# seung-lab/chunkflow

Measured on AMD Instinct MI355X. Metric: output_voxels_per_sec, higher is better.
Workload: dtype f32; 1 GPU; config2-512cube-rsunet-affinity; batch_size=12, engine=rsunet

## Files before the change

chunkflow_amd/csrc/updown.hip:

```cpp
#include <hip/hip_runtime.h>
#include <hip/hip_bf16.h>

#include <algorithm>

#include "cfx_internal.h"

namespace {

typedef __hip_bfloat16 cfx_bf16;

template <typename T>
__device__ __forceinline__ float ldf(const T* p);
template <>
__device__ __forceinline__ float ldf<float>(const float* p) { return *p; }
template <>
__device__ __forceinline__ float ldf<cfx_bf16>(const cfx_bf16* p) {
    return __bfloat162float(*p);
}
__device__ __forceinline__ float cvf(float v) { return v; }
__device__ __forceinline__ float cvf(cfx_bf16 v) {
    return __bfloat162float(v);
}

template <typename T>
struct vec4;
template <>
struct vec4<float> {
    typedef float type __attribute__((ext_vector_type(4)));
    static __device__ __forceinline__ float get(type v, int i) {
        return v[i];
    }
};
template <>
struct vec4<cfx_bf16> {
    typedef unsigned short type __attribute__((ext_vector_type(4)));
    static __device__ __forceinline__ float get(type v, int i) {
        return __bfloat162float(
            __hip_bfloat16(__hip_bfloat16_raw{(unsigned short)v[i]}));
    }
};
template <typename T>
__device__ __forceinline__ void stf(T* p, float v);
template <>
__device__ __forceinline__ void stf<float>(float* p, float v) { *p = v; }
template <>
__device__ __forceinline__ void stf<cfx_bf16>(cfx_bf16* p, float v) {
    *p = __float2bfloat16(v);
}

template <typename T>
__device__ __forceinline__ void stage_rows(
    float* s_in, const T* in, const long long* row_off, int rows, int xn,
    int xvalid, int C, int CPAD, int tid, int nthreads) {
    const int total = rows * xn * C;
    for (int idx = tid; idx < total; idx += nthreads) {
        const int c = idx % C;
        const int x = (idx / C) % xn;
        const int r = idx / (C * xn);
        const float v = x < xvalid
                            ? ldf(&in[row_off[r] + (long long)x * C + c])
                            : 0.f;
        s_in[(r * xn + x) * CPAD + c] = v;
    }
}

template <typename T, int XI>
__global__ __launch_bounds__(256, 2) void k_upconv2(
    const T* __restrict__ in, const T* __restrict__ wgt,
    const float* __restrict__ bias, T* __restrict__ out, int N, int D,
    int H, int W, int C, int K) {
    constexpr int PX = XI / 8;
    extern __shared__ float smem[];
    float* s_w = smem;
    float* s_in = smem + C * K * 4;
    const int CPAD = C | 1;
    const int tid = threadIdx.x;
    const int kslot = tid & 31;
    const int pslot = tid >> 5;

    for (int idx = tid; idx < C * K * 4; idx += 256) {
        const int q = idx & 3;
        const int k = (idx >> 2) % K;
        const int c = (idx >> 2) / K;
        s_w[(c * K + k) * 4 + q] = ldf(&wgt[(q * C + c) * K + k]);
    }

    const int nz = blockIdx.z;
    const int y = blockIdx.y;
    const int x0 = blockIdx.x * XI;
    const int xvalid = min(XI, W - x0);
    long long row_off[1] = {((((long long)nz * H) + y) * W + x0) * C};
    stage_rows(s_in, in, row_off, 1, XI, xvalid, C, CPAD, tid, 256);
    __syncthreads();

    const long long out_base =
        ((((long long)nz * 2 * H) + 2 * y) * 2 * W) * K;

    for (int k = kslot; k < K; k += 32) {
        const float bj = bias ? bias[k] : 0.f;
        float acc[PX][4];
#pragma unroll
        for (int p = 0; p < PX; ++p)
#pragma unroll
            for (int q = 0; q < 4; ++q) acc[p][q] = bj;
        for (int c = 0; c < C; ++c) {
            const float4 w4 =
                *reinterpret_cast<const float4*>(&s_w[(c * K + k) * 4]);
#pragma unroll
            for (int p = 0; p < PX; ++p) {
                const float v = s_in[(pslot + p * 8) * CPAD + c];
                acc[p][0] += v * w4.x;
                acc[p][1] += v * w4.y;
                acc[p][2] += v * w4.z;
                acc[p][3] += v * w4.w;
            }
        }
#pragma unroll
        for (int p = 0; p < PX; ++p) {
            const int xi = x0 + pslot + p * 8;
            if (xi >= W) continue;
            T* op = out + out_base + (long long)2 * xi * K + k;
            stf(op, acc[p][0]);
            stf(op + K, acc[p][1]);
            stf(op + (long long)2 * W * K, acc[p][2]);
            stf(op + (long long)2 * W * K + K, acc[p][3]);
        }
    }
}


constexpr int UM_NW = 4;

typedef float um_f32x4 __attribute__((ext_vector_type(4)));

template <int NT, bool SKIP>
__global__ __launch_bounds__(UM_NW * 64) void k_upconv2_mfma(
    const float* __restrict__ in, const float* __restrict__ wgt,
    const float* __restrict__ bias, const float* __restrict__ skip,
    float* __restrict__ out, int W, int C, int xtiles, int ntiles) {
    constexpr int K = 4 * NT;
    constexpr int N4 = 4 * K;
    constexpr int BS = N4 + 4;
    constexpr int RUN4 = 2 * NT;
    extern __shared__ __attribute__((aligned(16))) float um_smem[];
    const int S = C >> 2;
    const int tid = threadIdx.x;
    const int lane = tid & 63;
    const int wave = __builtin_amdgcn_readfirstlane(tid >> 6);
    float* s_w = um_smem;
    float* s_b = um_smem + C * N4 + wave * (16 * BS);

    for (int idx = tid; idx < C * N4; idx += UM_NW * 64) {
        const int l = idx & 63;
        const int st = idx >> 6;
        const int t = st % NT;
        const int s = st / NT;
        const int c = 4 * s + (l >> 4);
        const int col = 16 * t + (l & 15);
        const int q = col / K;
        s_w[idx] = wgt[(q * C + c) * K + (col - q * K)];
    }
    __syncthreads();

    const int ai = lane & 15;
    const int akk = lane >> 4;
    float bj[NT];
#pragma unroll
    for (int t = 0; t < NT; ++t)
        bj[t] = bias ? bias[(16 * t + ai) % K] : 0.f;

    auto piece = [&](int it, int& py, int& i, int& j4) {
        const int f = it * 64 + lane;
        py = f >= 16 * RUN4;
        const int rem = f - py * (16 * RUN4);
        i = rem / RUN4;
        j4 = rem - i * RUN4;
    };
    auto a_loads = [&](int tile, float (&a)[16]) {
        const int xt = tile % xtiles;
        const long long row = tile / xtiles;
        const int x0 = xt * 16;
        const int ilast = min(16, W - x0) - 1;
        const float* ip = in + (row * W + x0) * C;
        const unsigned ao = min(ai, ilast) * C + akk;
#pragma unroll
        for (int s = 0; s < 16; ++s) a[s] = ip[ao + 4u * min(s, S - 1)];
    };
    auto skip_loads = [&](int tile, um_f32x4 (&sv)[NT]) {
        const int xt = tile % xtiles;
        const long long row = tile / xtiles;
        const int x0 = xt * 16;
        const int ilast = min(16, W - x0) - 1;
        const float* sp = skip + (2 * row * 2 * W + 2 * x0) * K;
#pragma unroll
        for (int it = 0; it < NT; ++it) {
            int py, i, j4;
            piece(it, py, i, j4);
            const unsigned so =
                py * (2 * W * K) + min(i, ilast) * (2 * K) + 4 * j4;
            sv[it] = *reinterpret_cast<const um_f32x4*>(sp + so);
        }
    };

    auto do_tile = [&](int tile, int next, const float (&a)[16],
                       float (&a2)[16]) {
        um_f32x4 sv[NT];
        if (SKIP) skip_loads(tile, sv);
        a_loads(next, a2);
        __builtin_amdgcn_sched_barrier(0);
        um_f32x4 acc[NT];
#pragma unroll
        for (int t = 0; t < NT; ++t)
            acc[t] = um_f32x4{bj[t], bj[t], bj[t], bj[t]};
#pragma unroll
        for (int s = 0; s < 16; ++s) {
            if (s >= S) break;
#pragma unroll
            for (int t = 0; t < NT; ++t)
                acc[t] = __builtin_amdgcn_mfma_f32_16x16x4f32(
                    a[s], s_w[(s * NT + t) * 64 + lane], acc[t], 0, 0, 0);
        }
#pragma unroll
        for (int t = 0; t < NT; ++t)
#pragma unroll
            for (int r = 0; r < 4; ++r)
                s_b[(akk * 4 + r) * BS + 16 * t + ai] = acc[t][r];
        __builtin_amdgcn_wave_barrier();

        const int xt = tile % xtiles;
        const long long row = tile / xtiles;
        const int x0 = xt * 16;
        const int nvalid = min(16, W - x0);
        float* op = out + (2 * row * 2 * W + 2 * x0) * K;
        um_f32x4 v[NT];
#pragma unroll
        for (int it = 0; it < NT; ++it) {
            int py, i, j4;
            piece(it, py, i, j4);
            v[it] = *reinterpret_cast<const um_f32x4*>(
                &s_b[i * BS + py * (2 * K) + 4 * j4]);
            if (SKIP) v[it] += sv[it];
        }
        __builtin_amdgcn_sched_barrier(0);
#pragma unroll
        for (int it = 0; it < NT; ++it) {
            int py, i, j4;
            piece(it, py, i, j4);
            const unsigned oo = py * (2 * W * K) + i * (2 * K) + 4 * j4;
            if (nvalid == 16 || i < nvalid)
                *reinterpret_cast<um_f32x4*>(op + oo) = v[it];
        }
        __builtin_amdgcn_wave_barrier();
    };

    const int stride = gridDim.x * UM_NW;
    int tile = blockIdx.x * UM_NW + wave;
    if (tile >= ntiles) return;
    float a0[16], a1[16];
    a_loads(tile, a0);
    while (true) {
        do_tile(tile, min(tile + stride, ntiles - 1), a0, a1);
        tile += stride;
        if (tile >= ntiles) break;
        do_tile(tile, min(tile + stride, ntiles - 1), a1, a0);
        tile += stride;
        if (tile >= ntiles) break;
    }
}

template <typename T, int XO>
__global__ __launch_bounds__(256, 2) void k_downconv2(
    const T* __restrict__ in, const T* __restrict__ wgt,
    const float* __restrict__ bias, T* __restrict__ out, int N, int D,
    int H, int W, int C, int K) {
    constexpr int PX = XO / 8;
    extern __shared__ float smem[];
    float* s_w = smem;
    float* s_in = smem + C * K * 4;
    const int CPAD = C | 1;
    const int tid = threadIdx.x;
    const int kslot = tid & 31;
    const int pslot = tid >> 5;
    const int HO = H >> 1, WO = W >> 1;

    for (int idx = tid; idx < C * K * 4; idx += 256) {
        const int q = idx & 3;
        const int k = (idx >> 2) % K;
        const int c = (idx >> 2) / K;
        s_w[(c * K + k) * 4 + q] = ldf(&wgt[(q * C + c) * K + k]);
    }

    const int nz = blockIdx.z;
    const int y = blockIdx.y;
    const int x0 = blockIdx.x * XO;
    const int xvalid = min(2 * XO, W - 2 * x0);
    long long row_off[2] = {
        ((((long long)nz * H) + 2 * y) * W + 2 * x0) * C,
        ((((long long)nz * H) + 2 * y + 1) * W + 2 * x0) * C};
    stage_rows(s_in, in, row_off, 2, 2 * XO, xvalid, C, CPAD, tid, 256);
    __syncthreads();

    const long long out_row = (((long long)nz * HO) + y) * WO * K;

    for (int k = kslot; k < K; k += 32) {
        const float bj = bias ? bias[k] : 0.f;
        float acc[PX];
#pragma unroll
        for (int p = 0; p < PX; ++p) acc[p] = bj;
        for (int c = 0; c < C; ++c) {
            const float4 w4 =
                *reinterpret_cast<const float4*>(&s_w[(c * K + k) * 4]);
#pragma unroll
            for (int p = 0; p < PX; ++p) {
                const int xl = 2 * (pslot + p * 8);
                acc[p] += s_in[xl * CPAD + c] * w4.x;
                acc[p] += s_in[(xl + 1) * CPAD + c] * w4.y;
                acc[p] += s_in[(2 * XO + xl) * CPAD + c] * w4.z;
                acc[p] += s_in[(2 * XO + xl + 1) * CPAD + c] * w4.w;
            }
        }
#pragma unroll
        for (int p = 0; p < PX; ++p) {
            const int xo = x0 + pslot + p * 8;
            if (xo >= WO) continue;
            stf(&out[out_row + (long long)xo * K + k], acc[p]);
        }
    }
}

template <typename T, int XI, int KC>
__global__ __launch_bounds__(256, 2) void k_conv155_c1(
    const T* __restrict__ in, const T* __restrict__ wgt,
    const float* __restrict__ bias, T* __restrict__ out, int N, int D,
    int H, int W, int K_rt) {
    const int K = KC > 0 ? KC : K_rt;
    __shared__ float s_in[5][XI + 4];
    __shared__ float s_w[32 * 28];
    const int tid = threadIdx.x;
    const int nz = blockIdx.z;
    const int y = blockIdx.y;
    const int x0 = blockIdx.x * XI;

    const long long plane = (long long)nz * H;
    for (int idx = tid; idx < 5 * (XI + 4); idx += XI) {
        const int dy = idx / (XI + 4);
        const int xl = idx % (XI + 4);
        const int gy = y + dy - 2;
        const int gx = x0 + xl - 2;
        const bool ok = gy >= 0 && gy < H && gx >= 0 && gx < W;
        s_in[dy][xl] = ok ? ldf(&in[(plane + gy) * W + gx]) : 0.f;
    }
    for (int idx = tid; idx < K * 28; idx += XI) {
        const int t = idx % 28;
        const int k = idx / 28;
        s_w[idx] = t < 25 ? ldf(&wgt[k * 25 + t]) : 0.f;
    }
    __syncthreads();

    const int gx = x0 + tid;
    if (gx >= W) return;
    float v[25];
#pragma unroll
    for (int dy = 0; dy < 5; ++dy)
#pragma unroll
        for (int dx = 0; dx < 5; ++dx)
            v[dy * 5 + dx] = s_in[dy][tid + dx];
    T* op = out + (plane + y) * (long long)W * K + (long long)gx * K;
    if (KC > 0 && KC % 4 == 0) {
        typedef unsigned int uint2v __attribute__((ext_vector_type(2)));
        typedef float float2v __attribute__((ext_vector_type(2)));
#pragma unroll 1
        for (int k = 0; k < KC; k += 4) {
            float a0 = bias ? bias[k] : 0.f;
            float a1 = bias ? bias[k + 1] : 0.f;
            float a2 = bias ? bias[k + 2] : 0.f;
            float a3 = bias ? bias[k + 3] : 0.f;
#pragma unroll
            for (int t4 = 0; t4 < 24; t4 += 4) {
                const float4 w0 = *reinterpret_cast<const float4*>(
                    &s_w[k * 28 + t4]);
                const float4 w1 = *reinterpret_cast<const float4*>(
                    &s_w[(k + 1) * 28 + t4]);
                const float4 w2 = *reinterpret_cast<const float4*>(
                    &s_w[(k + 2) * 28 + t4]);
                const float4 w3 = *reinterpret_cast<const float4*>(
                    &s_w[(k + 3) * 28 + t4]);
                a0 += v[t4] * w0.x + v[t4 + 1] * w0.y + v[t4 + 2] * w0.z +
                      v[t4 + 3] * w0.w;
                a1 += v[t4] * w1.x + v[t4 + 1] * w1.y + v[t4 + 2] * w1.z +
                      v[t4 + 3] * w1.w;
                a2 += v[t4] * w2.x + v[t4 + 1] * w2.y + v[t4 + 2] * w2.z +
                      v[t4 + 3] * w2.w;
                a3 += v[t4] * w3.x + v[t4 + 1] * w3.y + v[t4 + 2] * w3.z +
                      v[t4 + 3] * w3.w;
            }
            a0 += v[24] * s_w[k * 28 + 24];
            a1 += v[24] * s_w[(k + 1) * 28 + 24];
            a2 += v[24] * s_w[(k + 2) * 28 + 24];
            a3 += v[24] * s_w[(k + 3) * 28 + 24];
            if (sizeof(T) == 2) {
                uint2v u;
                u.x = (unsigned)((__hip_bfloat16_raw)__float2bfloat16(
                          a0)).x |
                      ((unsigned)((__hip_bfloat16_raw)__float2bfloat16(
                           a1)).x << 16);
                u.y = (unsigned)((__hip_bfloat16_raw)__float2bfloat16(
                          a2)).x |
                      ((unsigned)((__hip_bfloat16_raw)__float2bfloat16(
                           a3)).x << 16);
                *reinterpret_cast<uint2v*>(reinterpret_cast<char*>(op) +
                                           (size_t)k * 2) = u;
            } else {
                float2v f01, f23;
                f01.x = a0;
                f01.y = a1;
                f23.x = a2;
                f23.y = a3;
                float2v* d =
                    reinterpret_cast<float2v*>(reinterpret_cast<char*>(op) +
                                               (size_t)k * 4);
                d[0] = f01;
                d[1] = f23;
            }
        }
    } else {
        for (int k = 0; k < K; ++k) {
            float acc = bias ? bias[k] : 0.f;
#pragma unroll
            for (int t4 = 0; t4 < 24; t4 += 4) {
                const float4 w4 =
                    *reinterpret_cast<const float4*>(&s_w[k * 28 + t4]);
                acc += v[t4] * w4.x + v[t4 + 1] * w4.y +
                       v[t4 + 2] * w4.z + v[t4 + 3] * w4.w;
            }
            acc += v[24] * s_w[k * 28 + 24];
            stf(&op[k], acc);
        }
    }
}

constexpr int CO_R = 6;
constexpr int CO_S = 60;
constexpr int CO_PS = 72;

typedef float co_f32x4 __attribute__((ext_vector_type(4)));

__device__ __forceinline__ unsigned short bf16_bits(float v) {
    return ((__hip_bfloat16_raw)__float2bfloat16(v)).x;
}

template <typename T>
__global__ __launch_bounds__(256, 2) void k_conv155_out_mfma(
    const T* __restrict__ in, const float* __restrict__ wfrag,
    const float* __restrict__ bias, T* __restrict__ out, int H, int W,
    int vec_ok) {
    constexpr int RS = CO_R + 4;
    constexpr int XS = 64;
    constexpr int CC = 28, C4 = CC / 4;
    constexpr int NV = RS * XS * C4;
    constexpr int PER = (NV + 255) / 256;
    constexpr int BATCH = 6;
    static_assert(CO_R * 16 * CO_PS * 4 <= RS * XS * CC * (int)sizeof(T),
                  "P bounce must fit over the input tile");
    __shared__ __attribute__((aligned(16))) T s_in[RS * XS * CC];
    float* s_p = reinterpret_cast<float*>(s_in);

    const int tid = threadIdx.x;
    const int wave = tid >> 6;
    const int lane = tid & 63;
    const int y0 = blockIdx.y * CO_R;
    const int x0 = blockIdx.x * CO_S;
    const long long plane = (long long)blockIdx.z * H;
    const int nout = min(CO_S, W - x0);
    const int ntile = (nout + 4 + 15) >> 4;

    float b[35];
#pragma unroll
    for (int s = 0; s < 35; ++s) b[s] = wfrag[s * 64 + lane];

    typedef typename vec4<T>::type tx4;
#pragma unroll 1
    for (int b0 = 0; b0 < PER; b0 += BATCH) {
        tx4 v[BATCH];
#pragma unroll
        for (int u = 0; u < BATCH; ++u) {
            const int idx = (b0 + u) * 256 + tid;
            const int r = idx / (XS * C4);
            const int rem = idx - r * (XS * C4);
            const int xl = rem / C4;
            const int c4 = rem - xl * C4;
            const int gy = y0 + r - 2;
            const int gx = x0 + xl - 2;
            const bool ok = b0 + u < PER && idx < NV && gy >= 0 &&
                            gy < H && gx >= 0 && gx < W &&
                            xl < ntile * 16;
            v[u] = ok ? *reinterpret_cast<const tx4*>(
                            &in[((plane + gy) * W + gx) * (long long)CC +
                                c4 * 4])
                      : tx4{};
        }
#pragma unroll
        for (int u = 0; u < BATCH; ++u) {
            const int idx = (b0 + u) * 256 + tid;
            if (b0 + u < PER && idx < NV)
                *reinterpret_cast<tx4*>(&s_in[idx * 4]) = v[u];
        }
    }
    __syncthreads();

    co_f32x4 acc[CO_R];
#pragma unroll
    for (int y = 0; y < CO_R; ++y) acc[y] = co_f32x4{0.f, 0.f, 0.f, 0.f};
    if (wave < ntile) {
        const T* abase = &s_in[(wave * 16 + (lane & 15)) * CC + (lane >> 4)];
#pragma unroll
        for (int r = 0; r < RS; ++r) {
            float a[C4];
#pragma unroll
            for (int s = 0; s < C4; ++s)
                a[s] = cvf(abase[r * XS * CC + s * 4]);
#pragma unroll
            for (int s = 0; s < C4; ++s)
#pragma unroll
                for (int dy = 0; dy < 5; ++dy) {
                    const int y = r - dy;
                    if (y >= 0 && y < CO_R)
                        acc[y] = __builtin_amdgcn_mfma_f32_16x16x4f32(
                            a[s], b[dy * C4 + s], acc[y], 0, 0, 0);
                }
        }
    }
    __syncthreads();

    if (wave < ntile) {
#pragma unroll
        for (int y = 0; y < CO_R; ++y)
            *reinterpret_cast<co_f32x4*>(
                &s_p[(y * 16 + (lane & 15)) * CO_PS + wave * 16 +
                     (lane >> 4) * 4]) = acc[y];
    }
    __syncthreads();

    if (tid >= CO_R * (CO_S / 4)) return;
    const int yl = tid / (CO_S / 4);
    const int q = tid - yl * (CO_S / 4);
    const int y = y0 + yl;
    const int gx = x0 + q * 4;
    if (y >= H || gx >= W) return;
    float o[4][3];
#pragma unroll
    for (int e = 0; e < 4; ++e)
#pragma unroll
        for (int k = 0; k < 3; ++k) o[e][k] = bias ? bias[k] : 0.f;
#pragma unroll
    for (int j = 0; j < 15; ++j) {
        const int dx = j / 3, k = j % 3;
        const float* pr = &s_p[(yl * 16 + j) * CO_PS + q * 4];
        const co_f32x4 lo = *reinterpret_cast<const co_f32x4*>(pr);
        const co_f32x4 hi = *reinterpret_cast<const co_f32x4*>(pr + 4);
        const float p8[8] = {lo[0], lo[1], lo[2], lo[3],
                             hi[0], hi[1], hi[2], hi[3]};
#pragma unroll
        for (int e = 0; e < 4; ++e) o[e][k] += p8[e + dx];
    }
    T* op = out + ((plane + y) * W + gx) * 3LL;
    if (vec_ok) {
        if (sizeof(T) == 2) {
            typedef unsigned co_u32x2 __attribute__((ext_vector_type(2)));
            unsigned short h[12];
#pragma unroll
            for (int i = 0; i < 12; ++i) h[i] = bf16_bits(o[i / 3][i % 3]);
#pragma unroll
            for (int i = 0; i < 3; ++i) {
                co_u32x2 u;
                u.x = h[4 * i] | ((unsigned)h[4 * i + 1] << 16);
                u.y = h[4 * i + 2] | ((unsigned)h[4 * i + 3] << 16);
                reinterpret_cast<co_u32x2*>(op)[i] = u;
            }
        } else {
#pragma unroll
            for (int i = 0; i < 3; ++i) {
                co_f32x4 f;
#pragma unroll
                for (int m = 0; m < 4; ++m)
                    f[m] = o[(4 * i + m) / 3][(4 * i + m) % 3];
                reinterpret_cast<co_f32x4*>(op)[i] = f;
            }
        }
    } else {
#pragma unroll
        for (int e = 0; e < 4; ++e)
            if (gx + e < W)
#pragma unroll
                for (int k = 0; k < 3; ++k) stf(&op[e * 3 + k], o[e][k]);
    }
}

__device__ __forceinline__ float bre_act(float v, int do_elu) {
    if (do_elu) {
        const float e = expm1f(v > 0.f ? 0.f : v);
        v = v > 0.f ? v : e;
    }
    return v;
}

template <bool VEC>
__global__ __launch_bounds__(256) void k_bias_res_elu(
    float* __restrict__ y, const float* __restrict__ bias,
    const float* __restrict__ res, long long total, int K, int do_elu) {
    const long long step = (long long)gridDim.x * 256;
    long long i = (long long)blockIdx.x * 256 + threadIdx.x;
    if (VEC) {
        const long long n4 = total >> 2;
        const int K4 = K >> 2;
        for (; i < n4; i += step) {
            const int k4 = (int)(i % K4);
            um_f32x4 v = reinterpret_cast<const um_f32x4*>(y)[i];
            if (bias) v += reinterpret_cast<const um_f32x4*>(bias)[k4];
            if (res) v += reinterpret_cast<const um_f32x4*>(res)[i];
#pragma unroll
            for (int e = 0; e < 4; ++e) v[e] = bre_act(v[e], do_elu);
            reinterpret_cast<um_f32x4*>(y)[i] = v;
        }
    } else {
        for (; i < total; i += step) {
            float v = y[i];
            if (bias) v += bias[(int)(i % K)];
            if (res) v += res[i];
            y[i] = bre_act(v, do_elu);
        }
    }
}

}

extern "C" int cfx_conv155_out(cfx_ctx* ctx, const void* in,
                               const float* wfrag, const float* bias,
                               void* out, int N, int D, int H, int W,
                               int C, int K, int is_bf16) {
    if (C != 28 || K != 3) {
        g_err = "cfx_conv155_out: only C == 28, K == 3 instantiated";
        return -1;
    }
    if ((long long)N * D > 65535) {
        g_err = "cfx_conv155_out: N * D <= 65535 supported";
        return -1;
    }
    hipEvent_t e0;
    if (prof_begin(ctx, &e0)) return -1;
    dim3 grid((W + CO_S - 1) / CO_S, (H + CO_R - 1) / CO_R,
              (unsigned)(N * D));
    const int vec_ok = W % 4 == 0 && ((size_t)out & 15) == 0;
    if (is_bf16)
        hipLaunchKernelGGL((k_conv155_out_mfma<cfx_bf16>), grid, dim3(256),
                           0, ctx->stream, (const cfx_bf16*)in, wfrag, bias,
                           (cfx_bf16*)out, H, W, vec_ok);
    else
        hipLaunchKernelGGL((k_conv155_out_mfma<float>), grid, dim3(256), 0,
                           ctx->stream, (const float*)in, wfrag, bias,
                           (float*)out, H, W, vec_ok);
    CFX_CHECK(hipGetLastError());
    double flops = 2.0 * 25.0 * C * K * (double)N * D * H * W;
    if (prof_end(ctx, e0, CFX_K_CONV_STREAM, flops)) return -1;
    return 0;
}

extern "C" int cfx_conv155_c1(cfx_ctx* ctx, const void* in, const void* wgt,
                              const float* bias, void* out, int N, int D,
                              int H, int W, int K, int is_bf16) {
    if (K > 32) {
        g_err = "cfx_conv155_c1: K <= 32 supported";
        return -1;
    }
    constexpr int XI = 256;
    dim3 grid((W + XI - 1) / XI, H, (unsigned)(N * D));
    hipEvent_t e0;
    if (prof_begin(ctx, &e0)) return -1;
    if (is_bf16 && K == 28)
        hipLaunchKernelGGL((k_conv155_c1<cfx_bf16, XI, 28>), grid,
                           dim3(XI), 0, ctx->stream, (const cfx_bf16*)in,
                           (const cfx_bf16*)wgt, bias, (cfx_bf16*)out, N,
                           D, H, W, K);
    else if (is_bf16)
        hipLaunchKernelGGL((k_conv155_c1<cfx_bf16, XI, 0>), grid,
                           dim3(XI), 0, ctx->stream, (const cfx_bf16*)in,
                           (const cfx_bf16*)wgt, bias, (cfx_bf16*)out, N,
                           D, H, W, K);
    else if (K == 28)
        hipLaunchKernelGGL((k_conv155_c1<float, XI, 28>), grid, dim3(XI),
                           0, ctx->stream, (const float*)in,
                           (const float*)wgt, bias, (float*)out, N, D, H,
                           W, K);
    else
        hipLaunchKernelGGL((k_conv155_c1<float, XI, 0>), grid, dim3(XI),
                           0, ctx->stream, (const float*)in,
                           (const float*)wgt, bias, (float*)out, N, D, H,
                           W, K);
    CFX_CHECK(hipGetLastError());
    double flops = 2.0 * 25.0 * K * (double)N * D * H * W;
    if (prof_end(ctx, e0, CFX_K_CONV_STREAM, flops)) return -1;
    return 0;
}

namespace {

size_t um_shmem(int C, int K) {
    return ((size_t)C * 4 * K + (size_t)UM_NW * 16 * (4 * K + 4)) *
           sizeof(float);
}

bool um_eligible(const void* in, const void* skip, const void* out, int N,
                 int D, int H, int W, int C, int K) {
    return C % 4 == 0 && K % 4 == 0 && C >= 4 && C <= 64 && K >= 4 &&
           K <= 48 && (((size_t)in | (size_t)skip | (size_t)out) & 15) == 0 &&
           (long long)N * D * H * ((W + 15) / 16) < (1LL << 31);
}

template <int NT, bool SKIP>
int um_launch_nt(cfx_ctx* ctx, const float* in, const float* wgt,
                 const float* bias, const float* skip, float* out, int W,
                 int C, int xtiles, int ntiles) {
    const size_t shmem = um_shmem(C, 4 * NT);
    if (shmem > 64 * 1024)
        CFX_CHECK(hipFuncSetAttribute(
            reinterpret_cast<const void*>(&k_upconv2_mfma<NT, SKIP>),
            hipFuncAttributeMaxDynamicSharedMemorySize, (int)shmem));
    int cus = 0;
    CFX_CHECK(hipDeviceGetAttribute(
        &cus, hipDeviceAttributeMultiprocessorCount, ctx->device));
    const int per_cu = (int)std::min<size_t>(8, (160 * 1024) / shmem);
    const int grid =
        std::min((ntiles + UM_NW - 1) / UM_NW, std::max(1, cus * per_cu));
    hipLaunchKernelGGL((k_upconv2_mfma<NT, SKIP>), dim3(grid),
                       dim3(UM_NW * 64), shmem, ctx->stream, in, wgt, bias,
                       skip, out, W, C, xtiles, ntiles);
    CFX_CHECK(hipGetLastError());
    return 0;
}

template <bool SKIP>
int um_launch(cfx_ctx* ctx, const float* in, const float* wgt,
              const float* bias, const float* skip, float* out, int N,
              int D, int H, int W, int C, int K) {
    const int xtiles = (W + 15) / 16;
    const int ntiles = N * D * H * xtiles;
    if (ntiles == 0) return 0;
    switch (K / 4) {
#define UM_CASE(NT)                                                         \
    case NT:                                                                \
        return um_launch_nt<NT, SKIP>(ctx, in, wgt, bias, skip, out, W, C,  \
                                      xtiles, ntiles);
        UM_CASE(1) UM_CASE(2) UM_CASE(3) UM_CASE(4) UM_CASE(5) UM_CASE(6)
        UM_CASE(7) UM_CASE(8) UM_CASE(9) UM_CASE(10) UM_CASE(11)
        UM_CASE(12)
#undef UM_CASE
    }
    g_err = "upconv mfma: K not instantiated";
    return -1;
}

}

extern "C" int cfx_upconv_2x2_add(cfx_ctx* ctx, const void* in,
                                  const void* wgt, const float* bias,
                                  const void* skip, void* out, int N, int D,
                                  int H, int W, int C, int K, int is_bf16) {
    if (!skip)
        return cfx_upconv_2x2(ctx, in, wgt, bias, out, N, D, H, W, C, K,
                              is_bf16);
    if (is_bf16) {
        g_err = "cfx_upconv_2x2_add: skip is f32 only";
        return -1;
    }
    if (!um_eligible(in, skip, out, N, D, H, W, C, K)) {
        g_err = "cfx_upconv_2x2_add: skip needs C % 4 == 0, K % 4 == 0, "
                "C <= 64, K <= 48 and 16-byte aligned tensors";
        return -1;
    }
    hipEvent_t e0;
    if (prof_begin(ctx, &e0)) return -1;
    if (um_launch<true>(ctx, (const float*)in, (const float*)wgt, bias,
                        (const float*)skip, (float*)out, N, D, H, W, C, K))
        return -1;
    double flops = 2.0 * 4.0 * C * K * (double)N * D * H * W;
    if (prof_end(ctx, e0, CFX_K_CONV_STREAM, flops)) return -1;
    return 0;
}

extern "C" int cfx_upconv_2x2(cfx_ctx* ctx, const void* in, const void* wgt,
                              const float* bias, void* out, int N, int D,
                              int H, int W, int C, int K, int is_bf16) {
    if (K > 64 || C > 64) {
        g_err = "cfx_upconv_2x2: C, K <= 64 supported";
        return -1;
    }
    if (!is_bf16 && um_eligible(in, nullptr, out, N, D, H, W, C, K)) {
        hipEvent_t e0;
        if (prof_begin(ctx, &e0)) return -1;
        if (um_launch<false>(ctx, (const float*)in, (const float*)wgt, bias,
                             nullptr, (float*)out, N, D, H, W, C, K))
            return -1;
        double flops = 2.0 * 4.0 * C * K * (double)N * D * H * W;
        if (prof_end(ctx, e0, CFX_K_CONV_STREAM, flops)) return -1;
        return 0;
    }
    constexpr int XI = 64;
    dim3 grid((W + XI - 1) / XI, H, (unsigned)(N * D));
    const size_t shmem =
        ((size_t)C * K * 4 + (size_t)XI * (C | 1)) * sizeof(float);
    hipEvent_t e0;
    if (prof_begin(ctx, &e0)) return -1;
    if (is_bf16)
        hipLaunchKernelGGL((k_upconv2<cfx_bf16, XI>), grid, dim3(256),
                           shmem, ctx->stream, (const cfx_bf16*)in,
                           (const cfx_bf16*)wgt, bias, (cfx_bf16*)out, N, D,
                           H, W, C, K);
    else
        hipLaunchKernelGGL((k_upconv2<float, XI>), grid, dim3(256), shmem,
                           ctx->stream, (const float*)in, (const float*)wgt,
                           bias, (float*)out, N, D, H, W, C, K);
    CFX_CHECK(hipGetLastError());
    double flops = 2.0 * 4.0 * C * K * (double)N * D * H * W;
    if (prof_end(ctx, e0, CFX_K_CONV_STREAM, flops)) return -1;
    return 0;
}

extern "C" int cfx_downconv_2x2(cfx_ctx* ctx, const void* in,
                                const void* wgt, const float* bias,
                                void* out, int N, int D, int H, int W,
                                int C, int K, int is_bf16) {
    if (K > 64 || C > 64) {
        g_err = "cfx_downconv_2x2: C, K <= 64 supported";
        return -1;
    }
    if ((H | W) & 1) {
        g_err = "cfx_downconv_2x2: H, W must be even";
        return -1;
    }
    constexpr int XO = 64;
    dim3 grid((W / 2 + XO - 1) / XO, H / 2, (unsigned)(N * D));
    const size_t shmem =
        ((size_t)C * K * 4 + (size_t)2 * 2 * XO * (C | 1)) * sizeof(float);
    hipEvent_t e0;
    if (prof_begin(ctx, &e0)) return -1;
    if (is_bf16)
        hipLaunchKernelGGL((k_downconv2<cfx_bf16, XO>), grid, dim3(256),
                           shmem, ctx->stream, (const cfx_bf16*)in,
                           (const cfx_bf16*)wgt, bias, (cfx_bf16*)out, N, D,
                           H, W, C, K);
    else
        hipLaunchKernelGGL((k_downconv2<float, XO>), grid, dim3(256), shmem,
                           ctx->stream, (const float*)in, (const float*)wgt,
                           bias, (float*)out, N, D, H, W, C, K);
    CFX_CHECK(hipGetLastError());
    double flops = 2.0 * 4.0 * C * K * (double)N * D * (H / 2) * (W / 2);
    if (prof_end(ctx, e0, CFX_K_CONV_STREAM, flops)) return -1;
    return 0;
}

extern "C" int cfx_bias_res_elu(cfx_ctx* ctx, float* y, const float* bias,
                                const float* res, long long nvox, int K,
                                int do_elu) {
    if (nvox < 0 || K < 1) {
        g_err = "cfx_bias_res_elu: nvox >= 0, K >= 1";
        return -1;
    }
    const long long total = nvox * K;
    if (total == 0) return 0;
    const bool vec =
        K % 4 == 0 &&
        (((size_t)y | (size_t)bias | (size_t)res) & 15) == 0;
    const long long items = vec ? total / 4 : total;
    const int grid = (int)std::min<long long>((items + 255) / 256, 256 * 16);
    if (vec)
        hipLaunchKernelGGL((k_bias_res_elu<true>), dim3(grid), dim3(256), 0,
                           ctx->stream, y, bias, res, total, K, do_elu);
    else
        hipLaunchKernelGGL((k_bias_res_elu<false>), dim3(grid), dim3(256), 0,
                           ctx->stream, y, bias, res, total, K, do_elu);
    CFX_CHECK(hipGetLastError());
    return 0;
}
```

Baseline: 116.6 million voxels/s.

## Use MFMA for the 1-channel input conv and add y-walking fp32 output conv

After: 119.1 million voxels/s, median of 6. +2.2%, better.

```diff
diff --git a/chunkflow_amd/csrc/updown.hip b/chunkflow_amd/csrc/updown.hip
--- a/chunkflow_amd/csrc/updown.hip
+++ b/chunkflow_amd/csrc/updown.hip
@@ -46,6 +46,10 @@
 template <>
 __device__ __forceinline__ void stf<cfx_bf16>(cfx_bf16* p, float v) {
     *p = __float2bfloat16(v);
+}
+
+__device__ __forceinline__ unsigned short bf16_bits(float v) {
+    return ((__hip_bfloat16_raw)__float2bfloat16(v)).x;
 }
 
 template <typename T>
@@ -328,114 +332,143 @@
     }
 }
 
-template <typename T, int XI, int KC>
-__global__ __launch_bounds__(256, 2) void k_conv155_c1(
+constexpr int CI_R = 8;
+constexpr int CI_S = 64;
+constexpr int CI_NW = CI_S / 16;
+constexpr int CI_LW = CI_S + 4;
+
+template <typename T>
+__global__ __launch_bounds__(CI_NW * 64) void k_conv155_in_mfma(
     const T* __restrict__ in, const T* __restrict__ wgt,
-    const float* __restrict__ bias, T* __restrict__ out, int N, int D,
-    int H, int W, int K_rt) {
-    const int K = KC > 0 ? KC : K_rt;
-    __shared__ float s_in[5][XI + 4];
-    __shared__ float s_w[32 * 28];
+    const float* __restrict__ bias, T* __restrict__ out, int H, int W,
+    int K, int nstrips, int nrows, int vec_ok) {
+    constexpr int NS = (CI_R + 4) * CI_LW;
+    constexpr int PER = (NS + CI_NW * 64 - 1) / (CI_NW * 64);
+    __shared__ float s_in[NS];
+    __shared__ __attribute__((aligned(16))) float s_bounce[CI_NW][16 * 32];
+
     const int tid = threadIdx.x;
-    const int nz = blockIdx.z;
-    const int y = blockIdx.y;
-    const int x0 = blockIdx.x * XI;
-
-    const long long plane = (long long)nz * H;
-    for (int idx = tid; idx < 5 * (XI + 4); idx += XI) {
-        const int dy = idx / (XI + 4);
-        const int xl = idx % (XI + 4);
-        const int gy = y + dy - 2;
+    const int lane = tid & 63;
+    const int wave = __builtin_amdgcn_readfirstlane(tid >> 6);
+    const int ai = lane & 15;
+    const int akk = lane >> 4;
+    const int strip = (int)blockIdx.x % nstrips;
+    const int rest = (int)blockIdx.x / nstrips;
+    const int y0 = (rest % nrows) * CI_R;
+    const int x0 = strip * CI_S;
+    const long long plane = (long long)(rest / nrows) * H;
+
+    float v[PER];
+#pragma unroll
+    for (int u = 0; u < PER; ++u) {
+        const int idx = u * (CI_NW * 64) + tid;
+        const int r = idx / CI_LW;
+        const int xl = idx - r * CI_LW;
+        const int cy = min(max(y0 + r - 2, 0), H - 1);
+        const int cx = min(max(x0 + xl - 2, 0), W - 1);
+        v[u] = ldf(&in[(plane + cy) * W + cx]);
+    }
+    float b[7][2];
+#pragma unroll
+    for (int s = 0; s < 7; ++s)
+#pragma unroll
+        for (int t = 0; t < 2; ++t)
+            b[s][t] = ldf(&wgt[min(16 * t + ai, K - 1) * 25 +
+                               min(4 * s + akk, 24)]);
+    float bj[2];
+#pragma unroll
+    for (int t = 0; t < 2; ++t)
+        bj[t] = bias ? bias[min(16 * t + ai, K - 1)] : 0.f;
+#pragma unroll
+    for (int u = 0; u < PER; ++u) {
+        const int idx = u * (CI_NW * 64) + tid;
+        const int r = idx / CI_LW;
+        const int xl = idx - r * CI_LW;
+        const int gy = y0 + r - 2;
         const int gx = x0 + xl - 2;
         const bool ok = gy >= 0 && gy < H && gx >= 0 && gx < W;
-        s_in[dy][xl] = ok ? ldf(&in[(plane + gy) * W + gx]) : 0.f;
-    }
-    for (int idx = tid; idx < K * 28; idx += XI) {
-        const int t = idx % 28;
-        const int k = idx / 28;
-        s_w[idx] = t < 25 ? ldf(&wgt[k * 25 + t]) : 0.f;
-    }
+        if (idx < NS) s_in[idx] = ok ? v[u] : 0.f;
+    }
+#pragma unroll
+    for (int s = 0; s < 7; ++s)
+#pragma unroll
+        for (int t = 0; t < 2; ++t)
+            b[s][t] = 4 * s + akk < 25 && 16 * t + ai < K ? b[s][t] : 0.f;
+#pragma unroll
+    for (int t = 0; t < 2; ++t) bj[t] = 16 * t + ai < K ? bj[t] : 0.f;
     __syncthreads();
 
-    const int gx = x0 + tid;
-    if (gx >= W) return;
-    float v[25];
-#pragma unroll
-    for (int dy = 0; dy < 5; ++dy)
-#pragma unroll
-        for (int dx = 0; dx < 5; ++dx)
-            v[dy * 5 + dx] = s_in[dy][tid + dx];
-    T* op = out + (plane + y) * (long long)W * K + (long long)gx * K;
-    if (KC > 0 && KC % 4 == 0) {
-        typedef unsigned int uint2v __attribute__((ext_vector_type(2)));
-        typedef float float2v __attribute__((ext_vector_type(2)));
-#pragma unroll 1
-        for (int k = 0; k < KC; k += 4) {
-            float a0 = bias ? bias[k] : 0.f;
-            float a1 = bias ? bias[k + 1] : 0.f;
-            float a2 = bias ? bias[k + 2] : 0.f;
-            float a3 = bias ? bias[k + 3] : 0.f;
-#pragma unroll
-            for (int t4 = 0; t4 < 24; t4 += 4) {
-                const float4 w0 = *reinterpret_cast<const float4*>(
-                    &s_w[k * 28 + t4]);
-                const float4 w1 = *reinterpret_cast<const float4*>(
-                    &s_w[(k + 1) * 28 + t4]);
-                const float4 w2 = *reinterpret_cast<const float4*>(
-                    &s_w[(k + 2) * 28 + t4]);
-                const float4 w3 = *reinterpret_cast<const float4*>(
-                    &s_w[(k + 3) * 28 + t4]);
-                a0 += v[t4] * w0.x + v[t4 + 1] * w0.y + v[t4 + 2] * w0.z +
-                      v[t4 + 3] * w0.w;
-                a1 += v[t4] * w1.x + v[t4 + 1] * w1.y + v[t4 + 2] * w1.z +
-                      v[t4 + 3] * w1.w;
-                a2 += v[t4] * w2.x + v[t4 + 1] * w2.y + v[t4 + 2] * w2.z +
-                      v[t4 + 3] * w2.w;
-                a3 += v[t4] * w3.x + v[t4 + 1] * w3.y + v[t4 + 2] * w3.z +
-                      v[t4 + 3] * w3.w;
+    const int xt = x0 + 16 * wave;
+    if (xt >= W) return;
+    const int nvalid = min(16, W - xt);
+    const int rows = min(CI_R, H - y0);
+    float* s_b = s_bounce[wave];
+    int aoff[7];
+#pragma unroll
+    for (int s = 0; s < 7; ++s) {
+        const int t = min(4 * s + akk, 24);
+        aoff[s] = (t / 5) * CI_LW + (t % 5) + 16 * wave + ai;
+    }
+    const bool apad = 24 + akk >= 25;
+    auto a_reads = [&](int ry, float (&a)[7]) {
+#pragma unroll
+        for (int s = 0; s < 7; ++s) a[s] = s_in[ry * CI_LW + aoff[s]];
+        a[6] = apad ? 0.f : a[6];
+    };
+
+    float a[7];
+    a_reads(0, a);
+    for (int ry = 0; ry < rows; ++ry) {
+        um_f32x4 acc[2];
+#pragma unroll
+        for (int t = 0; t < 2; ++t)
+            acc[t] = um_f32x4{bj[t], bj[t], bj[t], bj[t]};
+#pragma unroll
+        for (int s = 0; s < 7; ++s)
+#pragma unroll
+            for (int t = 0; t < 2; ++t)
+                acc[t] = __builtin_amdgcn_mfma_f32_16x16x4f32(
+                    a[s], b[s][t], acc[t], 0, 0, 0);
+        a_reads(min(ry + 1, rows - 1), a);
+#pragma unroll
+        for (int t = 0; t < 2; ++t)
+            if (16 * t + ai < K) {
+#pragma unroll
+                for (int r = 0; r < 4; ++r)
+                    s_b[(akk * 4 + r) * K + 16 * t + ai] = acc[t][r];
             }
-            a0 += v[24] * s_w[k * 28 + 24];
-            a1 += v[24] * s_w[(k + 1) * 28 + 24];
-            a2 += v[24] * s_w[(k + 2) * 28 + 24];
-            a3 += v[24] * s_w[(k + 3) * 28 + 24];
-            if (sizeof(T) == 2) {
-                uint2v u;
-                u.x = (unsigned)((__hip_bfloat16_raw)__float2bfloat16(
-                          a0)).x |
-                      ((unsigned)((__hip_bfloat16_raw)__float2bfloat16(
-                           a1)).x << 16);
-                u.y = (unsigned)((__hip_bfloat16_raw)__float2bfloat16(
-                          a2)).x |
-                      ((unsigned)((__hip_bfloat16_raw)__float2bfloat16(
-                           a3)).x << 16);
-                *reinterpret_cast<uint2v*>(reinterpret_cast<char*>(op) +
-                                           (size_t)k * 2) = u;
-            } else {
-                float2v f01, f23;
-                f01.x = a0;
-                f01.y = a1;
-                f23.x = a2;
-                f23.y = a3;
-                float2v* d =
-                    reinterpret_cast<float2v*>(reinterpret_cast<char*>(op) +
-                                               (size_t)k * 4);
-                d[0] = f01;
-                d[1] = f23;
+        __builtin_amdgcn_wave_barrier();
+
+        T* op = out + ((plane + y0 + ry) * W + xt) * (long long)K;
+        if (vec_ok) {
+            const int npiece = nvalid * (K >> 2);
+            um_f32x4 p[2];
+#pragma unroll
+            for (int it = 0; it < 2; ++it)
+                p[it] = *reinterpret_cast<const um_f32x4*>(
+                    &s_b[4 * (it * 64 + lane)]);
+#pragma unroll
+            for (int it = 0; it < 2; ++it) {
+                const int f = it * 64 + lane;
+                if (f >= npiece) continue;
+                if (sizeof(T) == 2) {
+                    typedef unsigned ci_u32x2
+                        __attribute__((ext_vector_type(2)));
+                    ci_u32x2 h;
+                    h.x = bf16_bits(p[it][0]) |
+                          ((unsigned)bf16_bits(p[it][1]) << 16);
+                    h.y = bf16_bits(p[it][2]) |
+                          ((unsigned)bf16_bits(p[it][3]) << 16);
+                    reinterpret_cast<ci_u32x2*>(op)[f] = h;
+                } else {
+                    reinterpret_cast<um_f32x4*>(op)[f] = p[it];
+                }
             }
-        }
-    } else {
-        for (int k = 0; k < K; ++k) {
-            float acc = bias ? bias[k] : 0.f;
-#pragma unroll
-            for (int t4 = 0; t4 < 24; t4 += 4) {
-                const float4 w4 =
-                    *reinterpret_cast<const float4*>(&s_w[k * 28 + t4]);
-                acc += v[t4] * w4.x + v[t4 + 1] * w4.y +
-                       v[t4 + 2] * w4.z + v[t4 + 3] * w4.w;
-            }
-            acc += v[24] * s_w[k * 28 + 24];
-            stf(&op[k], acc);
-        }
+        } else {
+            const int ne = nvalid * K;
+            for (int e = lane; e < ne; e += 64) stf(&op[e], s_b[e]);
+        }
+        __builtin_amdgcn_wave_barrier();
     }
 }
 
@@ -444,10 +477,6 @@
 constexpr int CO_PS = 72;
 
 typedef float co_f32x4 __attribute__((ext_vector_type(4)));
-
-__device__ __forceinline__ unsigned short bf16_bits(float v) {
-    return ((__hip_bfloat16_raw)__float2bfloat16(v)).x;
-}
 
 template <typename T>
 __global__ __launch_bounds__(256, 2) void k_conv155_out_mfma(
@@ -596,6 +625,143 @@
     }
 }
 
+constexpr int CY_YS = 32;
+constexpr int CY_XO = 12;
+constexpr int CY_NW = 4;
+constexpr int CY_PS = 20;
+
+__global__ __launch_bounds__(CY_NW * 64, 4) void k_conv155_out_ywalk(
+    const float* __restrict__ in, const float* __restrict__ wfrag,
+    const float* __restrict__ bias, float* __restrict__ out, int H, int W,
+    int nxg, int nseg, int vec_ok) {
+    constexpr int CC = 28, C4 = CC / 4;
+    __shared__ __attribute__((aligned(16))) float s_bounce[CY_NW][16 * CY_PS];
+    __shared__ __attribute__((aligned(16))) float s_tile[CY_NW][16 * CC];
+    const int lane = threadIdx.x & 63;
+    const int wave = __builtin_amdgcn_readfirstlane(threadIdx.x >> 6);
+    const int ai = lane & 15, akk = lane >> 4;
+    const int xg = (int)blockIdx.x % nxg;
+    const int rest = (int)blockIdx.x / nxg;
+    const int y0 = (rest % nseg) * CY_YS;
+    const long long plane = (long long)(rest / nseg) * H;
+    const int xo = (xg * CY_NW + wave) * CY_XO;
+    if (xo >= W) return;
+    const int nout = min(CY_XO, W - xo);
+    const int ys = min(CY_YS, H - y0);
+    float* s_p = s_bounce[wave];
+    float* s_a = s_tile[wave];
+
+    float b[35];
+#pragma unroll
+    for (int s = 0; s < 35; ++s) b[s] = wfrag[s * 64 + lane];
+    float bk[3];
+#pragma unroll
+    for (int k = 0; k < 3; ++k) bk[k] = bias ? bias[k] : 0.f;
+
+    unsigned poff[2];
+    bool pok[2];
+#pragma unroll
+    for (int j = 0; j < 2; ++j) {
+        const int f = min(lane + 64 * j, 16 * C4 - 1);
+        const int gx = xo - 2 + f / C4;
+        pok[j] = gx >= 0 && gx < W;
+        poff[j] = min(max(gx, 0), W - 1) * CC + 4 * (f % C4);
+    }
+    auto a_loads = [&](int r, co_f32x4 (&v)[2]) {
+        const int cy = min(max(y0 - 2 + r, 0), H - 1);
+        const float* ip = in + (plane + cy) * W * CC;
+#pragma unroll
+        for (int j = 0; j < 2; ++j)
+            v[j] = *reinterpret_cast<const co_f32x4*>(ip + poff[j]);
+    };
+    auto a_stage = [&](const co_f32x4 (&v)[2]) {
+#pragma unroll
+        for (int j = 0; j < 2; ++j) {
+            co_f32x4 w;
+#pragma unroll
+            for (int e = 0; e < 4; ++e)
+                w[e] = pok[j] ? v[j][e] : 0.f;
+            *reinterpret_cast<co_f32x4*>(
+                &s_a[4 * min(lane + 64 * j, 16 * C4 - 1)]) = w;
+        }
+        __builtin_amdgcn_wave_barrier();
+    };
+    auto outval = [&](int e) {
+        const int x = e / 3, k = e - 3 * x;
+        float o = k == 0 ? bk[0] : (k == 1 ? bk[1] : bk[2]);
+#pragma unroll
+        for (int dx = 0; dx < 5; ++dx)
+            o += s_p[(dx * 3 + k) * CY_PS + x + dx];
+        return o;
+    };
+    auto finish = [&](const co_f32x4& p) {
+        *reinterpret_cast<co_f32x4*>(&s_p[ai * CY_PS + akk * 4]) = p;
+        __builtin_amdgcn_wave_barrier();
+        co_f32x4 o = co_f32x4{0.f, 0.f, 0.f, 0.f};
+        if (vec_ok) {
+            if (4 * lane < 3 * nout) {
+#pragma unroll
+                for (int m = 0; m < 4; ++m) o[m] = outval(4 * lane + m);
+            }
+        } else if (lane < 3 * nout) {
+            o[0] = outval(lane);
+        }
+        __builtin_amdgcn_wave_barrier();
+        return o;
+    };
+    auto put = [&](int yl, const co_f32x4& o) {
+        float* op = out + ((plane + y0 + yl) * W + xo) * 3LL;
+        if (vec_ok) {
+            if (4 * lane < 3 * nout)
+                reinterpret_cast<co_f32x4*>(op)[lane] = o;
+        } else if (lane < 3 * nout) {
+            op[lane] = o[0];
+        }
+    };
+
+    co_f32x4 acc[5];
+#pragma unroll
+    for (int q = 0; q < 5; ++q) acc[q] = co_f32x4{0.f, 0.f, 0.f, 0.f};
+    const int nrow = ys + 4;
+    float a[C4];
+    co_f32x4 an[2];
+    co_f32x4 pend = co_f32x4{0.f, 0.f, 0.f, 0.f};
+    a_loads(0, an);
+    a_stage(an);
+#pragma unroll 1
+    for (int r = 0; r < nrow; ++r) {
+        if (r >= 5) put(r - 5, pend);
+        a_loads(min(r + 1, nrow - 1), an);
+#pragma unroll
+        for (int s = 0; s < C4; ++s) a[s] = s_a[ai * CC + 4 * s + akk];
+        __builtin_amdgcn_wave_barrier();
+        const int gy = y0 - 2 + r;
+        if (r >= 4 && r < ys && gy < H) {
+#pragma unroll
+            for (int s = 0; s < C4; ++s)
+#pragma unroll
+                for (int dy = 0; dy < 5; ++dy)
+                    acc[4 - dy] = __builtin_amdgcn_mfma_f32_16x16x4f32(
+                        a[s], b[dy * C4 + s], acc[4 - dy], 0, 0, 0);
+        } else if (gy >= 0 && gy < H) {
+#pragma unroll
+            for (int dy = 0; dy < 5; ++dy) {
+                if (r - dy < 0 || r - dy >= ys) continue;
+#pragma unroll
+                for (int s = 0; s < C4; ++s)
+                    acc[4 - dy] = __builtin_amdgcn_mfma_f32_16x16x4f32(
+                        a[s], b[dy * C4 + s], acc[4 - dy], 0, 0, 0);
+            }
+        }
+        if (r >= 4) pend = finish(acc[0]);
+        a_stage(an);
+#pragma unroll
+        for (int q = 0; q < 4; ++q) acc[q] = acc[q + 1];
+        acc[4] = co_f32x4{0.f, 0.f, 0.f, 0.f};
+    }
+    put(ys - 1, pend);
+}
+
 __device__ __forceinline__ float bre_act(float v, int do_elu) {
     if (do_elu) {
         const float e = expm1f(v > 0.f ? 0.f : v);
@@ -646,19 +812,31 @@
         g_err = "cfx_conv155_out: N * D <= 65535 supported";
         return -1;
     }
+    if (!is_bf16 && (long long)N * D * ((H + CY_YS - 1) / CY_YS) *
+                            ((W + CY_NW * CY_XO - 1) / (CY_NW * CY_XO)) >
+                        0x7fffffffLL) {
+        g_err = "cfx_conv155_out: too many workgroups for one grid axis";
+        return -1;
+    }
     hipEvent_t e0;
     if (prof_begin(ctx, &e0)) return -1;
     dim3 grid((W + CO_S - 1) / CO_S, (H + CO_R - 1) / CO_R,
               (unsigned)(N * D));
     const int vec_ok = W % 4 == 0 && ((size_t)out & 15) == 0;
-    if (is_bf16)
+    if (is_bf16) {
         hipLaunchKernelGGL((k_conv155_out_mfma<cfx_bf16>), grid, dim3(256),
                            0, ctx->stream, (const cfx_bf16*)in, wfrag, bias,
                            (cfx_bf16*)out, H, W, vec_ok);
-    else
-        hipLaunchKernelGGL((k_conv155_out_mfma<float>), grid, dim3(256), 0,
-                           ctx->stream, (const float*)in, wfrag, bias,
-                           (float*)out, H, W, vec_ok);
+    } else {
+        const int nxg = (W + CY_NW * CY_XO - 1) / (CY_NW * CY_XO);
+        const int nseg = (H + CY_YS - 1) / CY_YS;
+        const long long nwg = (long long)N * D * nseg * nxg;
+        if (nwg > 0)
+            hipLaunchKernelGGL(k_conv155_out_ywalk, dim3((unsigned)nwg),
+                               dim3(CY_NW * 64), 0, ctx->stream,
+                               (const float*)in, wfrag, bias, (float*)out, H,
+                               W, nxg, nseg, vec_ok);
+    }
     CFX_CHECK(hipGetLastError());
     double flops = 2.0 * 25.0 * C * K * (double)N * D * H * W;
     if (prof_end(ctx, e0, CFX_K_CONV_STREAM, flops)) return -1;
@@ -672,30 +850,33 @@
         g_err = "cfx_conv155_c1: K <= 32 supported";
         return -1;
     }
-    constexpr int XI = 256;
-    dim3 grid((W + XI - 1) / XI, H, (unsigned)(N * D));
+    if (K < 1 || N < 0 || D < 0 || H < 1 || W < 1) {
+        g_err = "cfx_conv155_c1: K >= 1, N, D >= 0, H, W >= 1";
+        return -1;
+    }
+    const int nstrips = (W + CI_S - 1) / CI_S;
+    const int nrows = (H + CI_R - 1) / CI_R;
+    const long long nwg = (long long)N * D * nrows * nstrips;
+    if (nwg > 0x7fffffffLL) {
+        g_err = "cfx_conv155_c1: N * D * ceil(H/8) * ceil(W/64) < 2^31 "
+                "supported";
+        return -1;
+    }
+    if (nwg == 0) return 0;
+    const int vec_ok = K % 4 == 0 && ((size_t)out & 15) == 0;
     hipEvent_t e0;
     if (prof_begin(ctx, &e0)) return -1;
-    if (is_bf16 && K == 28)
-        hipLaunchKernelGGL((k_conv155_c1<cfx_bf16, XI, 28>), grid,
-                           dim3(XI), 0, ctx->stream, (const cfx_bf16*)in,
-                           (const cfx_bf16*)wgt, bias, (cfx_bf16*)out, N,
-                           D, H, W, K);
-    else if (is_bf16)
-        hipLaunchKernelGGL((k_conv155_c1<cfx_bf16, XI, 0>), grid,
-                           dim3(XI), 0, ctx->stream, (const cfx_bf16*)in,
-                           (const cfx_bf16*)wgt, bias, (cfx_bf16*)out, N,
-                           D, H, W, K);
-    else if (K == 28)
-        hipLaunchKernelGGL((k_conv155_c1<float, XI, 28>), grid, dim3(XI),
-                           0, ctx->stream, (const float*)in,
-                           (const float*)wgt, bias, (float*)out, N, D, H,
-                           W, K);
+    if (is_bf16)
+        hipLaunchKernelGGL((k_conv155_in_mfma<cfx_bf16>),
+                           dim3((unsigned)nwg), dim3(CI_NW * 64), 0,
+                           ctx->stream, (const cfx_bf16*)in,
+                           (const cfx_bf16*)wgt, bias, (cfx_bf16*)out, H, W,
+                           K, nstrips, nrows, vec_ok);
     else
-        hipLaunchKernelGGL((k_conv155_c1<float, XI, 0>), grid, dim3(XI),
-                           0, ctx->stream, (const float*)in,
-                           (const float*)wgt, bias, (float*)out, N, D, H,
-                           W, K);
+        hipLaunchKernelGGL((k_conv155_in_mfma<float>), dim3((unsigned)nwg),
+                           dim3(CI_NW * 64), 0, ctx->stream,
+                           (const float*)in, (const float*)wgt, bias,
+                           (float*)out, H, W, K, nstrips, nrows, vec_ok);
     CFX_CHECK(hipGetLastError());
     double flops = 2.0 * 25.0 * K * (double)N * D * H * W;
     if (prof_end(ctx, e0, CFX_K_CONV_STREAM, flops)) return -1;
```
